# Samirez/Visual_odometry

Hardware: AMD Instinct MI355X
Metric: frame-pairs/sec (1280x720, 2000 ORB feats) (higher is better)
Workload: dtype u8+f32+f64; 1 GPU; seeded synthetic 1280x720 drone flight (256 distinct rendered views, closed loop), 2000 ORB features/frame, 8 levels = BASELINE config 2; chunk of 257 consecutive frames -> 256 pairs (k, k+1) per GPU per step, each frame detected once; detector=orb, distinct_rendered_frames=256, pair_stride=1, contexts_per_gpu=3, keypoint_order=cv2, poly_solver=fast, matcher=crosscheck, matcher_kernel=mfma_fp4, ransac=5-point, conf 0.99, 1 px, seed 2^64-1, <=1000 iters, parallelism=single GPU, pairs_ok_last_step=256

## Files before the change

visual_odometry_amd/csrc/orb_kernels.hip:

```cpp
#include "vo_internal.h"
#include <type_traits>
#include <float.h>
#include <stdlib.h>

__constant__ int8_t c_pattern[256 * 4] = {
#include "orb_pattern.inc"
};
__constant__ int c_umax[16] = {15, 15, 15, 15, 14, 14, 14, 13, 13, 12, 11, 10, 9, 8, 6, 3};
__constant__ int c_gauss7[7] = {18, 34, 49, 55, 49, 34, 18};


typedef short vo_s16x2 __attribute__((ext_vector_type(2)));
typedef unsigned short vo_u16x2 __attribute__((ext_vector_type(2)));
__device__ __forceinline__ uint32_t pk_sub16(uint32_t a, uint32_t b)
{
    return __builtin_bit_cast(uint32_t, __builtin_bit_cast(vo_s16x2, a) - __builtin_bit_cast(vo_s16x2, b));
}
__device__ __forceinline__ uint32_t pk_add16(uint32_t a, uint32_t b)
{
    return __builtin_bit_cast(uint32_t, __builtin_bit_cast(vo_s16x2, a) + __builtin_bit_cast(vo_s16x2, b));
}
__device__ __forceinline__ uint32_t pk_min16(uint32_t a, uint32_t b)
{
    return __builtin_bit_cast(uint32_t, __builtin_elementwise_min(__builtin_bit_cast(vo_s16x2, a), __builtin_bit_cast(vo_s16x2, b)));
// ... 642 lines not shown
        for (int i = lane; i < FT_SCH * (FAST_TW + 2); i += 64) {
            const int gr = i / (FAST_TW + 2), cx = 3 + i % (FAST_TW + 2);
            const int gx = x0 - 4 + cx, gy = y0 - 1 + gr;
            if (gx < xlo || gx > xhi || gy < gylo || gy > gyhi) continue;
            s_sc[gr * FT_SCW + cx] = (uint8_t)fast_score_or_zero(s_px + (gr + 3) * FT_PXW + 12 + cx, t);
        }
        __syncthreads();
        uint8_t* s_out = s_px;
        for (int i = lane; i < FAST_TH * FAST_TW; i += 64) {
            const int ty = i / FAST_TW, tx = i % FAST_TW;
            const uint8_t* c = s_sc + (ty + 1) * FT_SCW + 4 + tx;
            const int sv = c[0];
            const bool win = sv && sv > c[-1] && sv > c[1] && sv > c[-FT_SCW - 1] && sv > c[-FT_SCW] && sv > c[-FT_SCW + 1] &&
                             sv > c[FT_SCW - 1] && sv > c[FT_SCW] && sv > c[FT_SCW + 1];
            s_out[i] = win ? (uint8_t)sv : 0;
            const int gx = x0 + tx, gy = y0 + ty;
            const bool keep = win && gx >= g.edge && gx < lv.w - g.edge && gy >= g.edge && gy < lv.h - g.edge;
            if (keep) atomicAdd(&hist[((size_t)f * VO_MAX_LEVELS + l) * 256 + sv], 1u);
            if (!DENSE) {
                const unsigned long long m = __ballot(keep);
                const int slot = nw + (int)__builtin_amdgcn_mbcnt_hi((uint32_t)(m >> 32), __builtin_amdgcn_mbcnt_lo((uint32_t)m, 0u));
                if (keep) my_list[slot] = ((uint32_t)sv << 16) | ((uint32_t)ty << 8) | (uint32_t)tx;
                nw += (int)__popcll(m);
            }
        }
        __syncthreads();
        for (int i = lane; i < FAST_TH * FAST_TW; i += 64) s_sc[(i / FAST_TW + 1) * FT_SCW + 4 + i % FAST_TW] = s_out[i];
        __syncthreads();
    }
    if (!DENSE) {
        FT_STAT(4, nw);
        if (lane == 0) tile_count[(size_t)f * g.ftiles_total + bid] = nw;
        return;
    }
#pragma unroll
    for (int i = lane; i < FAST_TH * (FAST_TW / 16); i += 64) {
        const int ty = i / (FAST_TW / 16), c16 = i % (FAST_TW / 16);
        const int gy = y0 + ty, gx = x0 + 16 * c16;
        const uint32_t* c = (const uint32_t*)(s_sc + (ty + 1) * FT_SCW + 4 + 16 * c16);
        if (gy < lv.h && gx < lv.stride)
            *(uint4*)(score + (size_t)f * g.frame_bytes + lv.off + (size_t)gy * lv.stride + gx) = make_uint4(c[0], c[1], c[2], c[3]);
    }
}

static_assert((FAST_TH * FAST_TW) % 64 == 0, "the dense fallback appends with full-wave ballots");
void launch_fast(hipStream_t s, const uint8_t* pyr, uint8_t* score, uint32_t* hist, const PyrGeom& g, int F,
                 uint32_t* tile_list, int* tile_count)
{
    if (tile_list) { if (g.ftiles_total > 0) hipLaunchKernelGGL(k_fast<false>, dim3(g.ftiles_total, F), dim3(64), 0, s, pyr, score, hist, g, tile_list, tile_count); }
    else hipLaunchKernelGGL(k_fast<true>, dim3(g.dtiles_total, F), dim3(64), 0, s, pyr, score, hist, g, tile_list, tile_count);
}


__global__ __launch_bounds__(64) void k_sel_threshold(PyrGeom g, FrameFeat ff, int* thr)
{
    const int l = blockIdx.x, f = blockIdx.y, lane = threadIdx.x;
    const LevelGeom lv = g.lv[l];
    const int want = g.score_type == 0 ? 2 * lv.quota : lv.quota;
    const uint32_t* h = ff.hist + ((size_t)f * VO_MAX_LEVELS + l) * 256;
    uint32_t c[4];
    int own = 0;
#pragma unroll
    for (int k = 0; k < 4; k++) { c[k] = h[255 - 4 * lane - k]; own += (int)c[k]; }
    int inc = own;
#pragma unroll
    for (int d = 1; d < 64; d <<= 1) { int v = __shfl_up(inc, d, 64); if (lane >= d) inc += v; }
    int acc = inc - own, T = 0;
#pragma unroll
    for (int k = 0; k < 4; k++) {
        acc += (int)c[k];
        const int score = 255 - 4 * lane - k;
        if (T == 0 && acc >= want && score >= 1) T = score;
    }
    const unsigned long long found = __ballot(T != 0);
    int result = 1;
    if (found) result = __shfl(T, __ffsll((long long)found) - 1, 64);
    if (want <= 0 || lv.w <= 2 * g.edge || lv.h <= 2 * g.edge) result = 256;
    if (lane == 0) {
        thr[f * VO_MAX_LEVELS + l] = result;
        if (result > 255) ff.cand_count[f * VO_MAX_LEVELS + l] = 0;
    }
}

template <bool EMIT>
__global__ __launch_bounds__(64) void k_sel_rows(const uint32_t* tile_list, const int* tile_count, PyrGeom g, FrameFeat ff,
                                                 const int* thr, int* chunk_count)
{
    extern __shared__ uint32_t s_sel[];
    const int f = blockIdx.y, lane = threadIdx.x;
    int l = 0;
    while (l + 1 < g.nlevels && (int)blockIdx.x >= g.lv[l + 1].sel_chunk_base) l++;
    const LevelGeom lv = g.lv[l];
    const int chunk = blockIdx.x - lv.sel_chunk_base;
    const int T = thr[f * VO_MAX_LEVELS + l];
    int* my_count = chunk_count + (size_t)f * g.sel_chunks_total + blockIdx.x;
    const int nchunks = (l + 1 < g.nlevels ? g.lv[l + 1].sel_chunk_base : g.sel_chunks_total) - lv.sel_chunk_base;
    if (T > 255) {
        if (!EMIT && lane == 0) *my_count = 0;
        if (EMIT && chunk == 0 && lane == 0) ff.cand_count[f * VO_MAX_LEVELS + l] = 0;
        return;
    }
    const size_t tile0 = (size_t)f * g.ftiles_total + lv.ftile_base + (size_t)chunk * lv.ftiles_x;
    if (!EMIT) {
        int n = 0;
        for (int t = 0; t < lv.ftiles_x; t++) {
            const int cnt = min(tile_count[tile0 + t], FT_LISTCAP);
            const uint32_t* lst = tile_list + (tile0 + t) * FT_LISTCAP;
            for (int j0 = 0; j0 < cnt; j0 += 64) {
                const int j = j0 + lane;
                const uint32_t e = j < cnt ? lst[j] : 0u;
                n += (int)__popcll(__ballot(j < cnt && (int)(e >> 16) >= T));
            }
        }
        if (lane == 0) *my_count = n;
        return;
    }
    int base = 0;
    {
        const int* cc = chunk_count + (size_t)f * g.sel_chunks_total + lv.sel_chunk_base;
        for (int c = lane; c < chunk; c += 64) base += cc[c];
#pragma unroll
        for (int d = 32; d >= 1; d >>= 1) base += __shfl_xor(base, d, 64);
    }
    const int W32 = (lv.w + 31) >> 5, NW = FAST_TH * W32;
    uint32_t* s_bm = s_sel;
    uint32_t* s_pf = s_sel + NW;
    for (int i = lane; i < NW; i += 64) s_bm[i] = 0u;
    __syncthreads();
    for (int t = 0; t < lv.ftiles_x; t++) {
        const int cnt = min(tile_count[tile0 + t], FT_LISTCAP);
        const uint32_t* lst = tile_list + (tile0 + t) * FT_LISTCAP;
        for (int j = lane; j < cnt; j += 64) {
            const uint32_t e = lst[j];
            if ((int)(e >> 16) >= T) { const uint32_t gx = (uint32_t)(lv.fox + t * FAST_TW) + (e & 255u); atomicOr(&s_bm[((e >> 8) & 255u) * W32 + (gx >> 5)], 1u << (gx & 31u)); }
        }
    }
    __syncthreads();
    int n;
    {
        const int per = (NW + 63) / 64, w0 = lane * per, w1 = min(NW, w0 + per);
        int own = 0;
        for (int wd = w0; wd < w1; wd++) own += __popc(s_bm[wd]);
        int inc = own;
#pragma unroll
        for (int d = 1; d < 64; d <<= 1) { const int v = __shfl_up(inc, d, 64); if (lane >= d) inc += v; }
        n = __shfl(inc, 63, 64);
        int acc = inc - own;
        for (int wd = w0; wd < w1; wd++) { s_pf[wd] = (uint32_t)acc; acc += __popc(s_bm[wd]); }
    }
    __syncthreads();
    bool overflow = false;
    uint32_t* out_pos = ff.cand_pos + (size_t)f * g.cand_total + lv.cand_off;
    float* out_resp = ff.cand_resp + (size_t)f * g.cand_total + lv.cand_off;
    for (int t = 0; t < lv.ftiles_x; t++) {
        const int cnt = min(tile_count[tile0 + t], FT_LISTCAP);
        const uint32_t* lst = tile_list + (tile0 + t) * FT_LISTCAP;
        for (int j = lane; j < cnt; j += 64) {
            const uint32_t e = lst[j];
            if ((int)(e >> 16) >= T) {
                const uint32_t ly = (e >> 8) & 255u, gx = (uint32_t)(lv.fox + t * FAST_TW) + (e & 255u);
                const int wd = (int)(ly * W32 + (gx >> 5));
                const int pos = base + (int)s_pf[wd] + __popc(s_bm[wd] & ((1u << (gx & 31u)) - 1u));
                if (pos < lv.cand_cap) { out_pos[pos] = (((uint32_t)(lv.foy + chunk * FAST_TH) + ly) << 16) | gx; out_resp[pos] = (float)(e >> 16); }
                else overflow = true;
            }
        }
    }
    if (overflow) atomicOr(&ff.flags[f], 1);
    if (chunk == nchunks - 1 && lane == 0) ff.cand_count[f * VO_MAX_LEVELS + l] = min(base + n, lv.cand_cap);
}

static size_t sel_bitmap_bytes(const PyrGeom& g)
{
    int w = 0;
    for (int l = 0; l < g.nlevels; l++) w = g.lv[l].w > w ? g.lv[l].w : w;
    return (size_t)2 * FAST_TH * ((w + 31) / 32) * 4;
}

void launch_select_fast(hipStream_t s, const PyrGeom& g, FrameFeat ff, int F, int* thr, int* chunk_count,
                        const uint32_t* tile_list, const int* tile_count)
{
    hipLaunchKernelGGL(k_sel_threshold, dim3(g.nlevels, F), dim3(64), 0, s, g, ff, thr);
    if (g.sel_chunks_total <= 0) return;
    hipLaunchKernelGGL(k_sel_rows<false>, dim3(g.sel_chunks_total, F), dim3(64), 0, s, tile_list, tile_count, g, ff, thr, chunk_count);
    hipLaunchKernelGGL(k_sel_rows<true>, dim3(g.sel_chunks_total, F), dim3(64), sel_bitmap_bytes(g), s, tile_list, tile_count, g, ff, thr, chunk_count);
}

void launch_all_winners(hipStream_t s, const PyrGeom& g, FrameFeat ff, const Cv2Buf& cb, int F, const uint32_t* tile_list, const int* tile_count)
{
    if (g.sel_chunks_total <= 0) return;
    PyrGeom ga = g;
    for (int l = 0; l < g.nlevels; l++) { ga.lv[l].cand_off = cb.all_off[l]; ga.lv[l].cand_cap = cb.all_cap[l]; }
    ga.cand_total = cb.all_total;
    FrameFeat fa = ff;
    fa.cand_pos = cb.all_pos; fa.cand_resp = cb.all_resp; fa.cand_count = cb.all_count;
    hipLaunchKernelGGL(k_sel_rows<false>, dim3(g.sel_chunks_total, F), dim3(64), 0, s, tile_list, tile_count, ga, fa, cb.ones, cb.chunk_count);
    hipLaunchKernelGGL(k_sel_rows<true>, dim3(g.sel_chunks_total, F), dim3(64), sel_bitmap_bytes(g), s, tile_list, tile_count, ga, fa, cb.ones, cb.chunk_count);
}

__global__ __launch_bounds__(256) void k_harris(const uint8_t* pyr, PyrGeom g, FrameFeat ff, int blocks_per_level)
{
    const int bid = xcd_tile(blockIdx.x, gridDim.x);
    const int f = bid / (blocks_per_level * g.nlevels), l = (bid / blocks_per_level) % g.nlevels;
    const int i = (bid % blocks_per_level) * 256 + threadIdx.x;
    const LevelGeom lv = g.lv[l];
    if (i >= min(ff.cand_count[f * VO_MAX_LEVELS + l], lv.cand_cap)) return;
    const size_t ci = (size_t)f * g.cand_total + lv.cand_off + i;
    const uint32_t pos = ff.cand_pos[ci];
    const int x0 = pos & 0xffff, y0 = pos >> 16, st = lv.stride;
    const uint8_t* img = pyr + (size_t)f * g.frame_bytes + lv.off + (size_t)(y0 - 4) * st + (x0 - 4);
    int dxr[9][7], sxr[9][7];
#pragma unroll
    for (int r = 0; r < 9; r++) {
        uint32_t w0, w1, w2;
        __builtin_memcpy(&w0, img + (size_t)r * st, 4);
        __builtin_memcpy(&w1, img + (size_t)r * st + 4, 4);
        __builtin_memcpy(&w2, img + (size_t)r * st + 8, 4);
        int px[9];
#pragma unroll
        for (int c = 0; c < 9; c++) px[c] = (int)(((c < 4 ? w0 : c < 8 ? w1 : w2) >> (8 * (c & 3))) & 255u);
#pragma unroll
        for (int c = 0; c < 7; c++) { dxr[r][c] = px[c + 2] - px[c]; sxr[r][c] = px[c] + 2 * px[c + 1] + px[c + 2]; }
    }
    int a = 0, b = 0, c = 0;
#pragma unroll
    for (int r = 1; r < 8; r++)
#pragma unroll
        for (int k = 0; k < 7; k++) {
            const int Ix = dxr[r - 1][k] + 2 * dxr[r][k] + dxr[r + 1][k];
            const int Iy = sxr[r + 1][k] - sxr[r - 1][k];
            a += Ix * Ix; b += Iy * Iy; c += Ix * Iy;
        }
    const float scale = 1.f / ((1 << 2) * 7 * 255.f);
    const float scale_sq_sq = scale * scale * scale * scale;
    ff.cand_resp[ci] = ((float)a * (float)b - (float)c * (float)c - 0.04f * ((float)a + (float)b) * ((float)a + (float)b)) * scale_sq_sq;
}

void launch_harris(hipStream_t s, const uint8_t* pyr, const PyrGeom& g, FrameFeat ff, int F)
{
    int maxcap = 0;
    for (int l = 0; l < g.nlevels; l++) maxcap = g.lv[l].cand_cap > maxcap ? g.lv[l].cand_cap : maxcap;
    const int bpl = (maxcap + 255) / 256;
    hipLaunchKernelGGL(k_harris, dim3(bpl * g.nlevels * F), dim3(256), 0, s, pyr, g, ff, bpl);
}

__device__ __forceinline__ uint32_t f2key(float v)
{
    uint32_t u = __float_as_uint(v);
    return (u & 0x80000000u) ? ~u : (u | 0x80000000u);
}
// ... 574 lines not shown
```

visual_odometry_amd/csrc/vo_api.hip:

```cpp
#include "vo_internal.h"
#include <float.h>
#include <math.h>
#include <stdio.h>
#include <stdlib.h>
#include <string.h>
#include <vector>
#include <algorithm>

#define MAX_EVENTS 160

struct DevList {
    struct Entry { void* p; bool pinned; };
    std::vector<Entry> ptrs;
    DevList() = default;
    DevList(const DevList&) = delete;
    DevList& operator=(DevList&& o) noexcept { if (this != &o) { release(); ptrs.swap(o.ptrs); } return *this; }
    ~DevList() { release(); }
    template <typename T> hipError_t alloc(T** p, size_t n) { return keep(hipMalloc((void**)p, (n ? n : 1) * sizeof(T)), (void**)p, false); }
    template <typename T> hipError_t alloc_pinned(T** p, size_t n)
    {
        return keep(hipHostMalloc((void**)p, (n ? n : 1) * sizeof(T), hipHostMallocDefault), (void**)p, true);
    }
    void release()
    {
// ... 252 lines not shown
        const double fv = fval;
        const int ival = cv_floor_d(fv);
        ofs[val] = 0; c1[val] = 0;
        if (ival >= 0 && ssize > 1) {
            if (ival < ssize - 1) {
                ofs[val] = ival;
                volatile double fr = fv - (double)ival;
                fr = fr * 256.0;
                c1[val] = (uint16_t)lrint((double)fr);
            } else {
                ofs[val] = ssize - 1;
                if (val < maxofst) maxofst = val;
            }
        } else if (val + 1 > minofst) minofst = val + 1;
    }
    *pmin = minofst; *pmax = maxofst;
}

static hipError_t alloc_pairbuf(DevList& mem, PairBuf& pb, int P, int cap, bool with_pose_mask)
{
    hipError_t e;
    const size_t pc = (size_t)P * cap;
    pb = PairBuf{};
#define A_(field, n) if ((e = mem.alloc(&pb.field, (n))) != hipSuccess) return e
    A_(slots, (size_t)P * 2); A_(nn_idx, pc * 2); A_(nn_dist, pc * 2); A_(nn_idx2, pc); A_(nn_dist2, pc);
    A_(m_q, pc); A_(m_t, pc); A_(m_d, pc); A_(m_count, (size_t)P);
    A_(px1, pc * 2); A_(px2, pc * 2); A_(xn1, pc * 2); A_(xn2, pc * 2);
    A_(mask, pc); A_(models, (size_t)P * 64 * 90);
    A_(in1, pc * 2); A_(in2, pc * 2); A_(ipx1, pc * 2); A_(ipx2, pc * 2);
    A_(res, (size_t)P); A_(X, pc * 4);
    if (with_pose_mask) { A_(pose_mask, pc); }
    if (const size_t n = nn_colkey_ints(P, cap)) { A_(nn_colkey, n); }
#undef A_
    return hipSuccess;
}

static int alloc_cv2(vo_ctx* ctx)
{
    if (ctx->cv2_ready) return VO_OK;
    const PyrGeom& g = ctx->g;
    Cv2Buf& cb = ctx->cv2;
    int off = 0;
    for (int l = 0; l < g.nlevels; l++) {
        const int px8 = g.lv[l].w * g.lv[l].h / 8 + 1024;
        cb.all_off[l] = off;
        cb.all_cap[l] = align_up(px8 > g.lv[l].cand_cap ? px8 : g.lv[l].cand_cap, 8);
        off += cb.all_cap[l];
    }
    cb.all_total = off;
    const size_t F = (size_t)ctx->max_frames, n = F * off;
    DevList& m = ctx->orb_mem;
    HIPCHK(m.alloc(&cb.all_pos, n)); HIPCHK(m.alloc(&cb.all_resp, n)); HIPCHK(m.alloc(&cb.work, n));
    HIPCHK(m.alloc(&cb.lpos, n)); HIPCHK(m.alloc(&cb.rpos, n));
    HIPCHK(m.alloc(&cb.all_count, F * VO_MAX_LEVELS)); HIPCHK(m.alloc(&cb.ones, F * VO_MAX_LEVELS));
    HIPCHK(m.alloc(&cb.chunk_count, F * (size_t)(g.sel_chunks_total + 1)));
    std::vector<int> ones(F * VO_MAX_LEVELS, 1);
    HIPCHK(hipMemcpy(cb.ones, ones.data(), ones.size() * sizeof(int), hipMemcpyHostToDevice));
    HIPCHK(hipMemset(cb.all_count, 0, F * VO_MAX_LEVELS * sizeof(int)));
    HIPCHK(hipDeviceSynchronize());
    ctx->cv2_ready = true;
    return VO_OK;
}

static void free_config(vo_ctx* c)
{
    c->configured = c->cv2_ready = false;
    c->orb_mem.release();
    c->pb_mem.release();
    c->pb_pairs = c->pb_cap = 0;
    clear_last_run(c);
}

static void comm_release(vo_ctx* ctx);
static int sift_frames_upload_enqueue(vo_ctx* ctx, const uint8_t* frames, int F, int row_stride, int64_t frame_stride, int first_slot);
static int sift_frames_detect_enqueue(vo_ctx* ctx, int first_slot, int F);

extern "C" int vo_version(void) { return 120; }

extern "C" int vo_create(int device_id, vo_ctx** out)
{
    if (!out) return VO_ERR_INVALID;
    *out = nullptr;
    int ndev = 0;
    if (hipGetDeviceCount(&ndev) != hipSuccess || device_id < 0 || device_id >= ndev) return VO_ERR_HIP;
    vo_ctx* ctx = new vo_ctx();
    ctx->device = device_id;
    if (hipSetDevice(device_id) != hipSuccess || hipStreamCreateWithFlags(&ctx->stream, hipStreamNonBlocking) != hipSuccess ||
        ctx->mem.alloc(&ctx->dK, 16) != hipSuccess) {
        delete ctx;
        return VO_ERR_HIP;
    }
    for (int i = 0; i < MAX_EVENTS; i++) { (void)hipEventCreate(&ctx->ev[i][0]); (void)hipEventCreate(&ctx->ev[i][1]); }
    ctx->ev_ready = true;
    (void)hipEventCreateWithFlags(&ctx->ev_det, hipEventDisableTiming);
    *out = ctx;
    return VO_OK;
}

extern "C" void vo_destroy(vo_ctx* ctx)
{
    if (!ctx) return;
    (void)hipSetDevice(ctx->device);
    (void)hipStreamSynchronize(ctx->stream);
    if (ctx->stream_jpg) { (void)hipStreamSynchronize(ctx->stream_jpg); (void)hipStreamDestroy(ctx->stream_jpg); }
    for (int i = 0; i < 2; i++) if (ctx->ev_jpg[i]) (void)hipEventDestroy(ctx->ev_jpg[i]);
    if (ctx->ev_ready) for (int i = 0; i < MAX_EVENTS; i++) { (void)hipEventDestroy(ctx->ev[i][0]); (void)hipEventDestroy(ctx->ev[i][1]); }
    if (ctx->ev_det) (void)hipEventDestroy(ctx->ev_det);
    comm_release(ctx);
    (void)hipStreamDestroy(ctx->stream);
    delete ctx;
// ... 208 lines not shown
    if (!ctx) return VO_ERR_INVALID;
    return frames_upload_enqueue(ctx, frames, F, row_stride, frame_stride, first_slot);
}

extern "C" int vo_frames_upload_color(vo_ctx* ctx, const uint8_t* frames, int F, int channels, int row_stride,
                                      int64_t frame_stride, int first_slot)
{
    if (!ctx) return VO_ERR_INVALID;
    if (channels == 1) return vo_frames_upload(ctx, frames, F, row_stride, frame_stride, first_slot);
    const Batch b = batch(ctx);
    if (!b.ready) FAIL(VO_ERR_NOT_CONFIGURED, "vo_batch_configure has not been called");
    if (channels != 3 && channels != 4) FAIL(VO_ERR_INVALID, "channels must be 1, 3 or 4");
    if (!frames || F < 0 || first_slot < 0 || first_slot + F > b.max_frames) FAIL(VO_ERR_INVALID, "slot range out of bounds");
    if (row_stride < b.w * channels || frame_stride < (int64_t)row_stride * b.h) FAIL(VO_ERR_INVALID, "strides too small");
    if (F == 0) return VO_OK;
    HIPCHK(hipSetDevice(ctx->device));
    const size_t per = (size_t)frame_stride;
    const int chunk = F < 64 ? F : 64;
    int rc = ctx->staging.grow(ctx, per * chunk); if (rc) return rc;
    for (int f0 = 0; f0 < F; f0 += chunk) {
        const int n = F - f0 < chunk ? F - f0 : chunk;
        HIPCHK(hipMemcpyAsync(ctx->staging.p, frames + (size_t)f0 * per, per * n, hipMemcpyHostToDevice, ctx->stream));
        StageTimer t(ctx, ST_GRAY);
        gray_into_slots(ctx, ctx->stream, ctx->staging.p, channels, row_stride, frame_stride, first_slot + f0, n);
    }
    HIPCHK(hipGetLastError());
    HIPCHK(hipStreamSynchronize(ctx->stream));
    if (ctx->prof) prof_collect(ctx);
    return VO_OK;
}

static int run_detect(vo_ctx* ctx, int first_slot, int F, int upto)
{
    const PyrGeom& g = ctx->g;
    hipStream_t s = ctx->stream;
    uint8_t* pyr = ctx->pyr + (size_t)first_slot * g.frame_bytes;
    uint8_t* blur = ctx->blur + (size_t)first_slot * g.frame_bytes;
    uint8_t* score = ctx->score + (size_t)first_slot * g.frame_bytes;
    FrameFeat ff = ctx->ff;
    ff.cand_pos += (size_t)first_slot * g.cand_total; ff.cand_resp += (size_t)first_slot * g.cand_total;
    ff.cand_count += (size_t)first_slot * VO_MAX_LEVELS;
    ff.kp_pos += (size_t)first_slot * g.kp_cap; ff.kp_level += (size_t)first_slot * g.kp_cap;
    ff.kp_resp += (size_t)first_slot * g.kp_cap; ff.kp_angle += (size_t)first_slot * g.kp_cap;
    ff.kp_xy += (size_t)first_slot * g.kp_cap * 2; ff.kp_size += (size_t)first_slot * g.kp_cap;
    ff.desc += (size_t)first_slot * g.kp_cap * 32;
    ff.kp_count += first_slot; ff.flags += first_slot;
    ff.hist += (size_t)first_slot * VO_MAX_LEVELS * 256;
    ff.tile_list += (size_t)first_slot * g.ftiles_total * FAST_LISTCAP; ff.tile_count += (size_t)first_slot * g.ftiles_total;
    {
        StageTimer t(ctx, ST_RESIZE);
        for (int l = 1; l < g.nlevels; l++) launch_resize(s, pyr, g, l, ctx->tabs[l], F);
    }
    if (upto < 1) return VO_OK;
    {
        StageTimer t(ctx, ST_MISC);
        HIPCHK(hipMemsetAsync(ff.hist, 0, (size_t)F * VO_MAX_LEVELS * 256 * sizeof(uint32_t), s));
        HIPCHK(hipMemsetAsync(ff.flags, 0, (size_t)F * sizeof(int), s));
        HIPCHK(hipMemsetAsync(ff.cand_count, 0, (size_t)F * VO_MAX_LEVELS * sizeof(int), s));
        if (ctx->kp_order == 1 && ctx->cv2_ready)
            HIPCHK(hipMemsetAsync(ctx->cv2.all_count + (size_t)first_slot * VO_MAX_LEVELS, 0, (size_t)F * VO_MAX_LEVELS * sizeof(int), s));
    }
    { StageTimer t(ctx, ST_FAST); launch_fast(s, pyr, score, ff.hist, g, F, upto < 2 ? nullptr : ff.tile_list, ff.tile_count); }
    if (upto < 2) return VO_OK;
    { StageTimer t(ctx, ST_SELECT_FAST); launch_select_fast(s, g, ff, F, ctx->sel_thr + (size_t)first_slot * VO_MAX_LEVELS, ctx->sel_chunk_count + (size_t)first_slot * g.sel_chunks_total, ff.tile_list, ff.tile_count); }
    if (g.score_type == 0) { StageTimer t(ctx, ST_HARRIS); launch_harris(s, pyr, g, ff, F); }
    { StageTimer t(ctx, ST_SELECT_HARRIS); launch_select_harris(s, g, ff, F, ctx->har_thr + (size_t)first_slot * VO_MAX_LEVELS, ctx->har_kept + (size_t)first_slot * VO_MAX_LEVELS); }
    if (ctx->kp_order == 1 && ctx->cv2_ready) {
        StageTimer t(ctx, ST_CV2_ORDER);
        Cv2Buf cb = ctx->cv2;
        const size_t fo = (size_t)first_slot;
        cb.all_pos += fo * cb.all_total; cb.all_resp += fo * cb.all_total; cb.work += fo * cb.all_total;
        cb.lpos += fo * cb.all_total; cb.rpos += fo * cb.all_total;
        cb.all_count += fo * VO_MAX_LEVELS; cb.ones += fo * VO_MAX_LEVELS; cb.chunk_count += fo * g.sel_chunks_total;
        launch_all_winners(s, g, ff, cb, F, ff.tile_list, ff.tile_count);
        launch_cv2_order(s, g, ff, cb, F, ctx->har_kept + fo * VO_MAX_LEVELS);
    }
    { StageTimer t(ctx, ST_ANGLE); launch_angle(s, pyr, g, ff, F); }
    { StageTimer t(ctx, ST_BLUR); launch_blur(s, pyr, blur, g, F); }
    {
        StageTimer t(ctx, ST_BRIEF);
        const int cx = desc_x_rows(g.kp_cap);
        ctx->descx_fp4 = nn_kernel(ctx, g.kp_cap) == NN_FP4;
        launch_brief(s, blur, g, ff, F, ctx->desc_x + (size_t)first_slot * cx * 256, cx, ctx->descx_fp4);
    }
    return VO_OK;
}

extern "C" int vo_batch_kp_capacity(vo_ctx* ctx)
{
    if (!ctx) return 0;
    const Batch b = batch(ctx);
    return b.ready ? b.kp_cap : 0;
}

extern "C" int vo_host_alloc(size_t bytes, void** out)
{
    if (!out) return VO_ERR_INVALID;
    *out = nullptr;
    return hipHostMalloc(out, bytes ? bytes : 1, hipHostMallocDefault) == hipSuccess ? VO_OK : VO_ERR_HIP;
}

extern "C" void vo_host_free(void* p)
{
    if (p) (void)hipHostFree(p);
}

static int detect_enqueue(vo_ctx* ctx, int first_slot, int F)
{
    const Batch b = batch(ctx);
    if (!b.ready) FAIL(VO_ERR_NOT_CONFIGURED, "vo_batch_configure has not been called");
    if (F < 0 || first_slot < 0 || first_slot + F > b.max_frames) FAIL(VO_ERR_INVALID, "slot range out of bounds");
    HIPCHK(hipSetDevice(ctx->device));
    if (F == 0) return VO_OK;
    if (b.sift) return sift_frames_detect_enqueue(ctx, first_slot, F);
    int rc = run_detect(ctx, first_slot, F, 2);
    if (rc) return rc;
    HIPCHK(hipGetLastError());
    return VO_OK;
}

extern "C" int vo_frames_detect_async(vo_ctx* ctx, int first_slot, int F)
{
    if (!ctx) return VO_ERR_INVALID;
    int rc = detect_enqueue(ctx, first_slot, F);
    if (rc) return rc;
    HIPCHK(hipEventRecord(ctx->ev_det, ctx->stream));
    ctx->ev_det_set = true;
    return VO_OK;
// ... 1841 lines not shown
```

visual_odometry_amd/csrc/vo_internal.h:

```cpp
#pragma once
#include <hip/hip_runtime.h>
#include <stdint.h>
#include "../../include/vo_hip.h"

enum {
    ST_GRAY = 0, ST_RESIZE, ST_FAST, ST_SELECT_FAST, ST_HARRIS, ST_SELECT_HARRIS, ST_ANGLE,
    ST_BLUR, ST_BRIEF, ST_MATCH_NN, ST_MATCH_SELECT, ST_RANSAC, ST_POSE, ST_TRIANGULATE,
    ST_MISC, ST_RESERVED, ST_SIFT_SCALE, ST_SIFT_EXTREMA, ST_SIFT_ORIENT, ST_SIFT_SORT, ST_SIFT_DESC, ST_CV2_ORDER, ST_GATHER, ST_RESERVED2
};

struct LevelGeom {
    int w, h, stride, off;
    int quota;
    float scale;
    int ftile_base, ftiles_x;
    int fox, foy;
    int dtile_base, dtiles_x;
    int btile_base, btiles_x;
    int cand_off, cand_cap;
    int sel_chunk_base;
};

struct PyrGeom {
    int nlevels, frame_bytes;
// ... 4 lines not shown
    LevelGeom lv[VO_MAX_LEVELS];
};

#define RS2_WW 256
#define RS2_WH 16
#ifndef RS2_WAVES
#define RS2_WAVES 4
#endif
#define RS2_THREADS (64 * RS2_WAVES)
#define RS2_TH (RS2_WAVES * RS2_WH)

struct ResizeTab {
    const int* xofs; const uint16_t* xc1;
    const int* yofs; const uint16_t* yc1;
    int min_x, max_x, min_y, max_y;
    int direct;
};

#ifndef FAST_TW
#define FAST_TW 112
#endif
#ifndef FAST_TH
#define FAST_TH 20
#endif
#define BLUR_TW 128
#ifndef BLUR_TH
#define BLUR_TH 48
#endif
#define FAST_LISTCAP ((FAST_TW / 2) * (FAST_TH / 2))

struct FrameFeat {
    uint32_t* cand_pos;
    float*    cand_resp;
    int*      cand_count;
    uint32_t* kp_pos;
    int*      kp_level;
    float*    kp_resp;
    float*    kp_angle;
    float*    kp_xy;
    float*    kp_size;
    uint8_t*  desc;
    int*      kp_count;
    int*      flags;
    uint32_t* hist;
    uint32_t* tile_list;
    int*      tile_count;
};

struct Cv2Buf {
    uint32_t* all_pos;
    float*    all_resp;
    int*      all_count;
    int*      chunk_count;
    int*      ones;
    uint2*    work;
    uint32_t* lpos;
    uint32_t* rpos;
    int all_off[VO_MAX_LEVELS], all_cap[VO_MAX_LEVELS], all_total;
};

struct PairBuf {
    int*      slots;
    int*      nn_idx;
    int*      nn_dist;
    int*      nn_idx2;
    int*      nn_dist2;
    int*      nn_colkey;
    int*      m_q;
    int*      m_t;
    float*    m_d;
    int*      m_count;
    double*   px1;
    double*   px2;
    double*   xn1;
    double*   xn2;
    uint8_t*  mask;
    double*   models;
    double*   in1;
    double*   in2;
    double*   ipx1;
    double*   ipx2;
    vo_pair_result* res;
    double*   X;
    uint8_t*  pose_mask;
};

struct RansacParams {
    double prob, thresh_px;
    int max_iters;
    uint64_t seed;
    double K[9];
    double dist_thresh;
    int dk_early;
};

const char* rccl_load(void);
const char* rccl_unique_id(uint8_t* id128);
const char* rccl_comm_init(void** comm, const uint8_t* id128, int rank, int world);
void rccl_comm_destroy(void* comm);
const char* rccl_comm_count(void* comm, int* n);
const char* rccl_all_gather_f64(void* comm, const double* send, double* recv, size_t count, hipStream_t s);
void launch_pack_records(hipStream_t s, const vo_pair_result* res, int B, int valid, double* rec);

void launch_gray(hipStream_t s, const uint8_t* src, int channels, int row_stride, int64_t frame_stride,
                 uint8_t* pyr, const PyrGeom& g, int F);
void launch_gray_plain(hipStream_t s, const uint8_t* src, int channels, int row_stride, int64_t frame_stride,
                       uint8_t* dst, int w, int h, int dstride, int64_t dframe, int F);
void launch_resize(hipStream_t s, uint8_t* pyr, const PyrGeom& g, int level, const ResizeTab& tab, int F);
void launch_fast(hipStream_t s, const uint8_t* pyr, uint8_t* score, uint32_t* hist, const PyrGeom& g, int F,
                 uint32_t* tile_list, int* tile_count);
void launch_select_fast(hipStream_t s, const PyrGeom& g, FrameFeat ff, int F, int* thr, int* chunk_count,
                        const uint32_t* tile_list, const int* tile_count);
void launch_harris(hipStream_t s, const uint8_t* pyr, const PyrGeom& g, FrameFeat ff, int F);
void launch_all_winners(hipStream_t s, const PyrGeom& g, FrameFeat ff, const Cv2Buf& cb, int F, const uint32_t* tile_list, const int* tile_count);
void launch_cv2_order(hipStream_t s, const PyrGeom& g, FrameFeat ff, Cv2Buf cb, int F, const int* kept);
void launch_retain_raw(hipStream_t s, const float* resp, int n, int n_points, uint2* a, uint32_t* lpos, uint32_t* rpos,
                       int* order, int* n_out);
void launch_select_harris(hipStream_t s, const PyrGeom& g, FrameFeat ff, int F, float* thr, int* kept);
void launch_angle(hipStream_t s, const uint8_t* pyr, const PyrGeom& g, FrameFeat ff, int F);
void launch_resize_linear(hipStream_t st, const uint8_t* src, int sw, int sh, int cn, int sstride, int64_t sframe,
                          uint8_t* dst, int dw, int dh, int dstride, int64_t dframe,
                          const int* xofs, const void* xa, const int* yofs, const void* yb, int area2, int F);
void launch_resize_area(hipStream_t st, const uint8_t* src, int cn, int sstride, uint8_t* dst, int dw, int dh, int dstride,
                        int isx, int isy, const int* xsi, const float* xal, const int* xst, const int* ysi, const float* yal, const int* yst);
#define SIFT_IMG_BORDER 5
#define SIFT_MAX_INTERP_STEPS 5
#define SIFT_MAX_OCT 16
#define SIFT_MAX_TAPS 64
struct SiftGeom {
    int nOct, nLayers;
    int w[SIFT_MAX_OCT], h[SIFT_MAX_OCT], stride[SIFT_MAX_OCT];
    size_t plane[SIFT_MAX_OCT];
    size_t goff[SIFT_MAX_OCT];
    size_t gframe;
};
struct SiftCand { int o, layer, r, c; };
struct SiftKp { float x, y, size, angle, response; int octave; };
struct SiftSurv { SiftKp kp; int o, layer, r, c; };
struct SiftExpTab { float tab[64]; };
int launch_sb_sweep_base(hipStream_t s, const uint8_t* img, int channels, int row_stride, int64_t frame_stride, int sw, int sh,
                         float* dstG, size_t g_fs, int stride, int F, const float* taps, int ntaps);
int launch_sb_sweep(hipStream_t s, const float* src, size_t src_fs, float* dstG, size_t g_fs, int w, int h, int stride, int F,
                    const float* taps, int ntaps, float* dstH = nullptr, size_t h_fs = 0, int hstride = 0, int hw = 0, int hh = 0);
void launch_sb_extrema(hipStream_t s, const SiftGeom& P, const float* gauss, int o, float threshold, SiftCand* cand, int* counts, int cap, int F);
void launch_sb_refine_orient(hipStream_t s, const SiftGeom& P, const float* gauss, const SiftCand* cand, int cand_cap, float contrastThr,
                             float edgeThr, float sigma, const SiftExpTab& E, SiftSurv* surv, int surv_cap, SiftKp* kps, int kp_cap, int* counts, int F, int waves);
void launch_sb_sort_emit(hipStream_t s, const SiftKp* kps, int kp_cap, int* counts, int* rank , void* rank_tmp , SiftKp* sorted,
                         SiftKp* out, int out_cap, int* out_count, int* out_flags, int cand_cap, int surv_cap, int F);
void launch_sb_descriptor(hipStream_t s, const SiftGeom& P, const float* gauss, const SiftKp* kps, int kp_cap, const int* counts, const SiftExpTab& E,
                          uint8_t* desc, uint8_t* desc_x, int cap_x, int* norms, int* flags, int first_slot, int F, int waves);
void launch_sb_unpack(hipStream_t s, const SiftKp* kps, int kp_cap, const int* counts, int first_slot, float* kp_xy, float* kp_size, float* kp_angle,
                      float* kp_resp, int* kp_oct, int* kp_count, const int* fin_count, const int* fin_flags, int* flags, int F);
void launch_match_nn_l2i8(hipStream_t s, const uint8_t* desc_x, const int* norms, const int* kp_count, int kp_cap, int cap_x, PairBuf pb, int P,
                          int dirs_mask, int knn2);

#include "jpeg_host.h"
void launch_jpeg_decode(hipStream_t s, const uint8_t* blob, JpegImage* imgs, const JpegTables* tabs, int F, uint8_t* clean, uint32_t* rst,
                        int16_t* coef, uint8_t* planes, uint8_t* out, int max_blocks, int max_w, int max_h, bool gray = false,
                        bool packed_tables = false ,
                        hipEvent_t coef_cleared = nullptr );

void launch_pnp_ransac(hipStream_t s, const double* obj, const double* img, const int* offsets, int B, const double* Kd,
                       int iterations, double reproj_err, double confidence, uint64_t seed, const uint32_t* rng_tab, int rng_n,
                       int refine_cv2, double* rvec, double* tvec, uint8_t* mask, int* ninl, int* status);
void launch_rodrigues(hipStream_t s, const double* in, int in_is_matrix, double* out);
void launch_blur(hipStream_t s, const uint8_t* pyr, uint8_t* blur, const PyrGeom& g, int F);
void launch_brief(hipStream_t s, const uint8_t* blur, const PyrGeom& g, FrameFeat ff, int F, uint8_t* desc_x, int cap_x, int fp4);
// ... 80 lines not shown
```

Baseline: 89070 frame-pairs/s.

## Fuse FAST threshold selection and all-winners compaction into shared select kernels

Result: faster. 91580 frame-pairs/s, median of 6 (+2.8%).

```diff
diff --git a/visual_odometry_amd/csrc/orb_kernels.hip b/visual_odometry_amd/csrc/orb_kernels.hip
--- a/visual_odometry_amd/csrc/orb_kernels.hip
+++ b/visual_odometry_amd/csrc/orb_kernels.hip
@@ -718,12 +718,9 @@
 }
 
 
-__global__ __launch_bounds__(64) void k_sel_threshold(PyrGeom g, FrameFeat ff, int* thr)
-{
-    const int l = blockIdx.x, f = blockIdx.y, lane = threadIdx.x;
-    const LevelGeom lv = g.lv[l];
+__device__ __forceinline__ int sel_threshold(const PyrGeom& g, const LevelGeom& lv, const uint32_t* h, int lane)
+{
     const int want = g.score_type == 0 ? 2 * lv.quota : lv.quota;
-    const uint32_t* h = ff.hist + ((size_t)f * VO_MAX_LEVELS + l) * 256;
     uint32_t c[4];
     int own = 0;
 #pragma unroll
@@ -742,126 +739,178 @@
     int result = 1;
     if (found) result = __shfl(T, __ffsll((long long)found) - 1, 64);
     if (want <= 0 || lv.w <= 2 * g.edge || lv.h <= 2 * g.edge) result = 256;
-    if (lane == 0) {
-        thr[f * VO_MAX_LEVELS + l] = result;
-        if (result > 255) ff.cand_count[f * VO_MAX_LEVELS + l] = 0;
-    }
-}
-
-template <bool EMIT>
-__global__ __launch_bounds__(64) void k_sel_rows(const uint32_t* tile_list, const int* tile_count, PyrGeom g, FrameFeat ff,
-                                                 const int* thr, int* chunk_count)
-{
-    extern __shared__ uint32_t s_sel[];
+    return __builtin_amdgcn_readfirstlane(result);
+}
+
+template <bool EMIT, bool ALL>
+__device__ __forceinline__ void sel_rows(const uint32_t* tile_list, const int* tile_count, const PyrGeom& g, const FrameFeat& ff,
+                                         int* thr, int* chunk_count, const Cv2Buf& cb, uint32_t* s_sel)
+{
     const int f = blockIdx.y, lane = threadIdx.x;
     int l = 0;
     while (l + 1 < g.nlevels && (int)blockIdx.x >= g.lv[l + 1].sel_chunk_base) l++;
     const LevelGeom lv = g.lv[l];
     const int chunk = blockIdx.x - lv.sel_chunk_base;
-    const int T = thr[f * VO_MAX_LEVELS + l];
-    int* my_count = chunk_count + (size_t)f * g.sel_chunks_total + blockIdx.x;
     const int nchunks = (l + 1 < g.nlevels ? g.lv[l + 1].sel_chunk_base : g.sel_chunks_total) - lv.sel_chunk_base;
-    if (T > 255) {
-        if (!EMIT && lane == 0) *my_count = 0;
-        if (EMIT && chunk == 0 && lane == 0) ff.cand_count[f * VO_MAX_LEVELS + l] = 0;
-        return;
-    }
+    const size_t cslot = (size_t)f * g.sel_chunks_total + blockIdx.x;
     const size_t tile0 = (size_t)f * g.ftiles_total + lv.ftile_base + (size_t)chunk * lv.ftiles_x;
     if (!EMIT) {
-        int n = 0;
-        for (int t = 0; t < lv.ftiles_x; t++) {
-            const int cnt = min(tile_count[tile0 + t], FT_LISTCAP);
-            const uint32_t* lst = tile_list + (tile0 + t) * FT_LISTCAP;
-            for (int j0 = 0; j0 < cnt; j0 += 64) {
-                const int j = j0 + lane;
-                const uint32_t e = j < cnt ? lst[j] : 0u;
-                n += (int)__popcll(__ballot(j < cnt && (int)(e >> 16) >= T));
+        const int T = sel_threshold(g, lv, ff.hist + ((size_t)f * VO_MAX_LEVELS + l) * 256, lane);
+        int n = 0, na = 0;
+        if (ALL || T <= 255)
+            for (int t = 0; t < lv.ftiles_x; t++) {
+                const int cnt = min(tile_count[tile0 + t], FT_LISTCAP);
+                const uint32_t* lst = tile_list + (tile0 + t) * FT_LISTCAP;
+                na += cnt;
+                for (int j0 = 0; j0 < cnt; j0 += 64) {
+                    const int j = j0 + lane;
+                    const uint32_t e = j < cnt ? lst[j] : 0u;
+                    n += (int)__popcll(__ballot(j < cnt && (int)(e >> 16) >= T));
+                }
             }
-        }
-        if (lane == 0) *my_count = n;
+        if (lane != 0) return;
+        chunk_count[cslot] = n;
+        if (ALL) cb.chunk_count[cslot] = na;
+        if (chunk == 0) thr[f * VO_MAX_LEVELS + l] = T;
+        if (blockIdx.x == 0) {
+            ff.flags[f] = 0;
+            for (int k = 0; k < g.nlevels; k++)
+                if ((k + 1 < g.nlevels ? g.lv[k + 1].sel_chunk_base : g.sel_chunks_total) == g.lv[k].sel_chunk_base) {
+                    ff.cand_count[f * VO_MAX_LEVELS + k] = 0;
+                    if (ALL) cb.all_count[f * VO_MAX_LEVELS + k] = 0;
+                }
+        }
         return;
     }
-    int base = 0;
+    const int T = thr[f * VO_MAX_LEVELS + l];
+    if (!ALL && T > 255) {
+        if (chunk == 0 && lane == 0) ff.cand_count[f * VO_MAX_LEVELS + l] = 0;
+        return;
+    }
+    int base = 0, abase = 0;
     {
-        const int* cc = chunk_count + (size_t)f * g.sel_chunks_total + lv.sel_chunk_base;
-        for (int c = lane; c < chunk; c += 64) base += cc[c];
-#pragma unroll
-        for (int d = 32; d >= 1; d >>= 1) base += __shfl_xor(base, d, 64);
+        const size_t c0 = (size_t)f * g.sel_chunks_total + lv.sel_chunk_base;
+        for (int c = lane; c < chunk; c += 64) { base += chunk_count[c0 + c]; if (ALL) abase += cb.chunk_count[c0 + c]; }
+#pragma unroll
+        for (int d = 32; d >= 1; d >>= 1) { base += __shfl_xor(base, d, 64); if (ALL) abase += __shfl_xor(abase, d, 64); }
     }
     const int W32 = (lv.w + 31) >> 5, NW = FAST_TH * W32;
     uint32_t* s_bm = s_sel;
     uint32_t* s_pf = s_sel + NW;
-    for (int i = lane; i < NW; i += 64) s_bm[i] = 0u;
+    uint32_t* s_abm = s_sel + 2 * NW;
+    uint32_t* s_apf = s_sel + 3 * NW;
+    for (int i = lane; i < NW; i += 64) { s_bm[i] = 0u; if (ALL) s_abm[i] = 0u; }
     __syncthreads();
     for (int t = 0; t < lv.ftiles_x; t++) {
         const int cnt = min(tile_count[tile0 + t], FT_LISTCAP);
         const uint32_t* lst = tile_list + (tile0 + t) * FT_LISTCAP;
         for (int j = lane; j < cnt; j += 64) {
             const uint32_t e = lst[j];
-            if ((int)(e >> 16) >= T) { const uint32_t gx = (uint32_t)(lv.fox + t * FAST_TW) + (e & 255u); atomicOr(&s_bm[((e >> 8) & 255u) * W32 + (gx >> 5)], 1u << (gx & 31u)); }
+            const bool kept = (int)(e >> 16) >= T;
+            if (ALL || kept) {
+                const uint32_t gx = (uint32_t)(lv.fox + t * FAST_TW) + (e & 255u), wd = ((e >> 8) & 255u) * W32 + (gx >> 5), bit = 1u << (gx & 31u);
+                if (ALL) atomicOr(&s_abm[wd], bit);
+                if (kept) atomicOr(&s_bm[wd], bit);
+            }
         }
     }
     __syncthreads();
-    int n;
+    int n, na = 0;
     {
         const int per = (NW + 63) / 64, w0 = lane * per, w1 = min(NW, w0 + per);
-        int own = 0;
-        for (int wd = w0; wd < w1; wd++) own += __popc(s_bm[wd]);
-        int inc = own;
-#pragma unroll
-        for (int d = 1; d < 64; d <<= 1) { const int v = __shfl_up(inc, d, 64); if (lane >= d) inc += v; }
+        int own = 0, aown = 0;
+        for (int wd = w0; wd < w1; wd++) { own += __popc(s_bm[wd]); if (ALL) aown += __popc(s_abm[wd]); }
+        int inc = own, ainc = aown;
+#pragma unroll
+        for (int d = 1; d < 64; d <<= 1) {
+            const int v = __shfl_up(inc, d, 64); if (lane >= d) inc += v;
+            if (ALL) { const int av = __shfl_up(ainc, d, 64); if (lane >= d) ainc += av; }
+        }
         n = __shfl(inc, 63, 64);
-        int acc = inc - own;
-        for (int wd = w0; wd < w1; wd++) { s_pf[wd] = (uint32_t)acc; acc += __popc(s_bm[wd]); }
+        if (ALL) na = __shfl(ainc, 63, 64);
+        int acc = inc - own, aacc = ainc - aown;
+        for (int wd = w0; wd < w1; wd++) {
+            s_pf[wd] = (uint32_t)acc; acc += __popc(s_bm[wd]);
+            if (ALL) { s_apf[wd] = (uint32_t)aacc; aacc += __popc(s_abm[wd]); }
+        }
     }
     __syncthreads();
     bool overflow = false;
     uint32_t* out_pos = ff.cand_pos + (size_t)f * g.cand_total + lv.cand_off;
     float* out_resp = ff.cand_resp + (size_t)f * g.cand_total + lv.cand_off;
+    uint32_t* all_pos = ALL ? cb.all_pos + (size_t)f * cb.all_total + cb.all_off[l] : nullptr;
+    float* all_resp = ALL ? cb.all_resp + (size_t)f * cb.all_total + cb.all_off[l] : nullptr;
+    const int all_cap = ALL ? cb.all_cap[l] : 0;
     for (int t = 0; t < lv.ftiles_x; t++) {
         const int cnt = min(tile_count[tile0 + t], FT_LISTCAP);
         const uint32_t* lst = tile_list + (tile0 + t) * FT_LISTCAP;
         for (int j = lane; j < cnt; j += 64) {
             const uint32_t e = lst[j];
-            if ((int)(e >> 16) >= T) {
+            const bool kept = (int)(e >> 16) >= T;
+            if (ALL || kept) {
                 const uint32_t ly = (e >> 8) & 255u, gx = (uint32_t)(lv.fox + t * FAST_TW) + (e & 255u);
                 const int wd = (int)(ly * W32 + (gx >> 5));
-                const int pos = base + (int)s_pf[wd] + __popc(s_bm[wd] & ((1u << (gx & 31u)) - 1u));
-                if (pos < lv.cand_cap) { out_pos[pos] = (((uint32_t)(lv.foy + chunk * FAST_TH) + ly) << 16) | gx; out_resp[pos] = (float)(e >> 16); }
-                else overflow = true;
+                const uint32_t below = (1u << (gx & 31u)) - 1u, key = (((uint32_t)(lv.foy + chunk * FAST_TH) + ly) << 16) | gx;
+                const float score = (float)(e >> 16);
+                if (ALL) {
+                    const int apos = abase + (int)s_apf[wd] + __popc(s_abm[wd] & below);
+                    if (apos < all_cap) { all_pos[apos] = key; all_resp[apos] = score; }
+                    else overflow = true;
+                }
+                if (kept) {
+                    const int pos = base + (int)s_pf[wd] + __popc(s_bm[wd] & below);
+                    if (pos < lv.cand_cap) { out_pos[pos] = key; out_resp[pos] = score; }
+                    else overflow = true;
+                }
             }
         }
     }
     if (overflow) atomicOr(&ff.flags[f], 1);
-    if (chunk == nchunks - 1 && lane == 0) ff.cand_count[f * VO_MAX_LEVELS + l] = min(base + n, lv.cand_cap);
-}
-
-static size_t sel_bitmap_bytes(const PyrGeom& g)
+    if (chunk == nchunks - 1 && lane == 0) {
+        ff.cand_count[f * VO_MAX_LEVELS + l] = min(base + n, lv.cand_cap);
+        if (ALL) cb.all_count[f * VO_MAX_LEVELS + l] = min(abase + na, all_cap);
+    }
+}
+
+template <bool EMIT>
+__global__ __launch_bounds__(64) void k_sel_rows(const uint32_t* tile_list, const int* tile_count, PyrGeom g, FrameFeat ff,
+                                                 int* thr, int* chunk_count)
+{
+    extern __shared__ uint32_t s_sel[];
+    sel_rows<EMIT, false>(tile_list, tile_count, g, ff, thr, chunk_count, Cv2Buf(), s_sel);
+}
+template <bool EMIT>
+__global__ __launch_bounds__(64) void k_sel_rows(const uint32_t* tile_list, const int* tile_count, PyrGeom g, FrameFeat ff,
+                                                 int* thr, int* chunk_count, Cv2Buf cb)
+{
+    extern __shared__ uint32_t s_sel[];
+    sel_rows<EMIT, true>(tile_list, tile_count, g, ff, thr, chunk_count, cb, s_sel);
+}
+
+static size_t sel_bitmap_bytes(const PyrGeom& g, bool all)
 {
     int w = 0;
     for (int l = 0; l < g.nlevels; l++) w = g.lv[l].w > w ? g.lv[l].w : w;
-    return (size_t)2 * FAST_TH * ((w + 31) / 32) * 4;
+    return (size_t)(all ? 4 : 2) * FAST_TH * ((w + 31) / 32) * 4;
 }
 
 void launch_select_fast(hipStream_t s, const PyrGeom& g, FrameFeat ff, int F, int* thr, int* chunk_count,
-                        const uint32_t* tile_list, const int* tile_count)
-{
-    hipLaunchKernelGGL(k_sel_threshold, dim3(g.nlevels, F), dim3(64), 0, s, g, ff, thr);
-    if (g.sel_chunks_total <= 0) return;
-    hipLaunchKernelGGL(k_sel_rows<false>, dim3(g.sel_chunks_total, F), dim3(64), 0, s, tile_list, tile_count, g, ff, thr, chunk_count);
-    hipLaunchKernelGGL(k_sel_rows<true>, dim3(g.sel_chunks_total, F), dim3(64), sel_bitmap_bytes(g), s, tile_list, tile_count, g, ff, thr, chunk_count);
-}
-
-void launch_all_winners(hipStream_t s, const PyrGeom& g, FrameFeat ff, const Cv2Buf& cb, int F, const uint32_t* tile_list, const int* tile_count)
-{
-    if (g.sel_chunks_total <= 0) return;
-    PyrGeom ga = g;
-    for (int l = 0; l < g.nlevels; l++) { ga.lv[l].cand_off = cb.all_off[l]; ga.lv[l].cand_cap = cb.all_cap[l]; }
-    ga.cand_total = cb.all_total;
-    FrameFeat fa = ff;
-    fa.cand_pos = cb.all_pos; fa.cand_resp = cb.all_resp; fa.cand_count = cb.all_count;
-    hipLaunchKernelGGL(k_sel_rows<false>, dim3(g.sel_chunks_total, F), dim3(64), 0, s, tile_list, tile_count, ga, fa, cb.ones, cb.chunk_count);
-    hipLaunchKernelGGL(k_sel_rows<true>, dim3(g.sel_chunks_total, F), dim3(64), sel_bitmap_bytes(g), s, tile_list, tile_count, ga, fa, cb.ones, cb.chunk_count);
+                        const uint32_t* tile_list, const int* tile_count, const Cv2Buf* cb)
+{
+    if (g.sel_chunks_total <= 0) {
+        (void)hipMemsetAsync(ff.flags, 0, (size_t)F * sizeof(int), s);
+        (void)hipMemsetAsync(ff.cand_count, 0, (size_t)F * VO_MAX_LEVELS * sizeof(int), s);
+        if (cb) (void)hipMemsetAsync(cb->all_count, 0, (size_t)F * VO_MAX_LEVELS * sizeof(int), s);
+        return;
+    }
+    const dim3 grid(g.sel_chunks_total, F);
+    if (cb) {
+        hipLaunchKernelGGL(k_sel_rows<false>, grid, dim3(64), 0, s, tile_list, tile_count, g, ff, thr, chunk_count, *cb);
+        hipLaunchKernelGGL(k_sel_rows<true>, grid, dim3(64), sel_bitmap_bytes(g, true), s, tile_list, tile_count, g, ff, thr, chunk_count, *cb);
+    } else {
+        hipLaunchKernelGGL(k_sel_rows<false>, grid, dim3(64), 0, s, tile_list, tile_count, g, ff, thr, chunk_count);
+        hipLaunchKernelGGL(k_sel_rows<true>, grid, dim3(64), sel_bitmap_bytes(g, false), s, tile_list, tile_count, g, ff, thr, chunk_count);
+    }
 }
 
 __global__ __launch_bounds__(256) void k_harris(const uint8_t* pyr, PyrGeom g, FrameFeat ff, int blocks_per_level)
diff --git a/visual_odometry_amd/csrc/vo_api.hip b/visual_odometry_amd/csrc/vo_api.hip
--- a/visual_odometry_amd/csrc/vo_api.hip
+++ b/visual_odometry_amd/csrc/vo_api.hip
@@ -328,10 +328,8 @@
     DevList& m = ctx->orb_mem;
     HIPCHK(m.alloc(&cb.all_pos, n)); HIPCHK(m.alloc(&cb.all_resp, n)); HIPCHK(m.alloc(&cb.work, n));
     HIPCHK(m.alloc(&cb.lpos, n)); HIPCHK(m.alloc(&cb.rpos, n));
-    HIPCHK(m.alloc(&cb.all_count, F * VO_MAX_LEVELS)); HIPCHK(m.alloc(&cb.ones, F * VO_MAX_LEVELS));
+    HIPCHK(m.alloc(&cb.all_count, F * VO_MAX_LEVELS));
     HIPCHK(m.alloc(&cb.chunk_count, F * (size_t)(g.sel_chunks_total + 1)));
-    std::vector<int> ones(F * VO_MAX_LEVELS, 1);
-    HIPCHK(hipMemcpy(cb.ones, ones.data(), ones.size() * sizeof(int), hipMemcpyHostToDevice));
     HIPCHK(hipMemset(cb.all_count, 0, F * VO_MAX_LEVELS * sizeof(int)));
     HIPCHK(hipDeviceSynchronize());
     ctx->cv2_ready = true;
@@ -646,28 +644,31 @@
         for (int l = 1; l < g.nlevels; l++) launch_resize(s, pyr, g, l, ctx->tabs[l], F);
     }
     if (upto < 1) return VO_OK;
+    const bool cv2 = ctx->kp_order == 1 && ctx->cv2_ready;
+    Cv2Buf cb = ctx->cv2;
+    if (cv2) {
+        const size_t fo = (size_t)first_slot;
+        cb.all_pos += fo * cb.all_total; cb.all_resp += fo * cb.all_total; cb.work += fo * cb.all_total;
+        cb.lpos += fo * cb.all_total; cb.rpos += fo * cb.all_total;
+        cb.all_count += fo * VO_MAX_LEVELS; cb.chunk_count += fo * g.sel_chunks_total;
+    }
     {
         StageTimer t(ctx, ST_MISC);
         HIPCHK(hipMemsetAsync(ff.hist, 0, (size_t)F * VO_MAX_LEVELS * 256 * sizeof(uint32_t), s));
-        HIPCHK(hipMemsetAsync(ff.flags, 0, (size_t)F * sizeof(int), s));
-        HIPCHK(hipMemsetAsync(ff.cand_count, 0, (size_t)F * VO_MAX_LEVELS * sizeof(int), s));
-        if (ctx->kp_order == 1 && ctx->cv2_ready)
-            HIPCHK(hipMemsetAsync(ctx->cv2.all_count + (size_t)first_slot * VO_MAX_LEVELS, 0, (size_t)F * VO_MAX_LEVELS * sizeof(int), s));
+        if (upto < 2) {
+            HIPCHK(hipMemsetAsync(ff.flags, 0, (size_t)F * sizeof(int), s));
+            HIPCHK(hipMemsetAsync(ff.cand_count, 0, (size_t)F * VO_MAX_LEVELS * sizeof(int), s));
+            if (cv2) HIPCHK(hipMemsetAsync(cb.all_count, 0, (size_t)F * VO_MAX_LEVELS * sizeof(int), s));
+        }
     }
     { StageTimer t(ctx, ST_FAST); launch_fast(s, pyr, score, ff.hist, g, F, upto < 2 ? nullptr : ff.tile_list, ff.tile_count); }
     if (upto < 2) return VO_OK;
-    { StageTimer t(ctx, ST_SELECT_FAST); launch_select_fast(s, g, ff, F, ctx->sel_thr + (size_t)first_slot * VO_MAX_LEVELS, ctx->sel_chunk_count + (size_t)first_slot * g.sel_chunks_total, ff.tile_list, ff.tile_count); }
+    { StageTimer t(ctx, ST_SELECT_FAST); launch_select_fast(s, g, ff, F, ctx->sel_thr + (size_t)first_slot * VO_MAX_LEVELS, ctx->sel_chunk_count + (size_t)first_slot * g.sel_chunks_total, ff.tile_list, ff.tile_count, cv2 ? &cb : nullptr); }
     if (g.score_type == 0) { StageTimer t(ctx, ST_HARRIS); launch_harris(s, pyr, g, ff, F); }
     { StageTimer t(ctx, ST_SELECT_HARRIS); launch_select_harris(s, g, ff, F, ctx->har_thr + (size_t)first_slot * VO_MAX_LEVELS, ctx->har_kept + (size_t)first_slot * VO_MAX_LEVELS); }
-    if (ctx->kp_order == 1 && ctx->cv2_ready) {
+    if (cv2) {
         StageTimer t(ctx, ST_CV2_ORDER);
-        Cv2Buf cb = ctx->cv2;
-        const size_t fo = (size_t)first_slot;
-        cb.all_pos += fo * cb.all_total; cb.all_resp += fo * cb.all_total; cb.work += fo * cb.all_total;
-        cb.lpos += fo * cb.all_total; cb.rpos += fo * cb.all_total;
-        cb.all_count += fo * VO_MAX_LEVELS; cb.ones += fo * VO_MAX_LEVELS; cb.chunk_count += fo * g.sel_chunks_total;
-        launch_all_winners(s, g, ff, cb, F, ff.tile_list, ff.tile_count);
-        launch_cv2_order(s, g, ff, cb, F, ctx->har_kept + fo * VO_MAX_LEVELS);
+        launch_cv2_order(s, g, ff, cb, F, ctx->har_kept + (size_t)first_slot * VO_MAX_LEVELS);
     }
     { StageTimer t(ctx, ST_ANGLE); launch_angle(s, pyr, g, ff, F); }
     { StageTimer t(ctx, ST_BLUR); launch_blur(s, pyr, blur, g, F); }
diff --git a/visual_odometry_amd/csrc/vo_internal.h b/visual_odometry_amd/csrc/vo_internal.h
--- a/visual_odometry_amd/csrc/vo_internal.h
+++ b/visual_odometry_amd/csrc/vo_internal.h
@@ -80,7 +80,6 @@
     float*    all_resp;
     int*      all_count;
     int*      chunk_count;
-    int*      ones;
     uint2*    work;
     uint32_t* lpos;
     uint32_t* rpos;
@@ -138,9 +137,8 @@
 void launch_fast(hipStream_t s, const uint8_t* pyr, uint8_t* score, uint32_t* hist, const PyrGeom& g, int F,
                  uint32_t* tile_list, int* tile_count);
 void launch_select_fast(hipStream_t s, const PyrGeom& g, FrameFeat ff, int F, int* thr, int* chunk_count,
-                        const uint32_t* tile_list, const int* tile_count);
+                        const uint32_t* tile_list, const int* tile_count, const Cv2Buf* cb);
 void launch_harris(hipStream_t s, const uint8_t* pyr, const PyrGeom& g, FrameFeat ff, int F);
-void launch_all_winners(hipStream_t s, const PyrGeom& g, FrameFeat ff, const Cv2Buf& cb, int F, const uint32_t* tile_list, const int* tile_count);
 void launch_cv2_order(hipStream_t s, const PyrGeom& g, FrameFeat ff, Cv2Buf cb, int F, const int* kept);
 void launch_retain_raw(hipStream_t s, const float* resp, int n, int n_points, uint2* a, uint32_t* lpos, uint32_t* rpos,
                        int* order, int* n_out);
```
